# jaak-s/BayesianDataFusion.jl

Hardware: AMD Instinct MI355X
Metric: Gibbs sweeps/sec (both entities) + test RMSE, MovieLens-1M D=32 (higher is better)
Workload: dtype f64; 1 GPU; BPMF MovieLens-1M 6040x3952, 500209 training ratings (500000 held out), D=32, alpha=1.5, step = rows of both entities + hyperpriors + test prediction update (one native call); BEFORE the --warmup steps the engine's set-up runs 60 ms of full iterations whose results are discarded (device_warmup_ms); num_latent=32, burnin=5, psamples=1985, parallelism=1 GPU

## Files before the change

### bayesiandatafusion.jl_amd/csrc/bdf_gibbs.hip

```cpp
#include "bdf_common.h"
#include <algorithm>
#include <chrono>
#include <cmath>
#include <cstdio>
#include <cstdlib>
#include <map>
#include <mutex>
#include <tuple>

struct bdf_gibbs {
    bdf_ctx *rows, *hyper, *pred;
    int D;
    struct Ent {
        bdf_gibbs_entity d;
        int cur;
        hipEvent_t ev_rows = nullptr, ev_hyper = nullptr;
        hipEvent_t ev_beta = nullptr;
        bool beta_recorded = false;
        bool hyper_recorded = false;
        uint32_t epoch = 0;
        uint32_t *done_dev = nullptr;
        uint32_t done_target = 0;
        hipEvent_t t_start = nullptr, t_stop = nullptr;
        unsigned long long *span = nullptr;
    };
    std::vector<Ent> ent;
    bdf_pairs *test;
    int32_t test_entity[BDF_MAX_MODES];
    double test_mean, clamp_lo, clamp_hi, class_cut;
    double *stats_dev;
    hipEvent_t ev_pred[3] = {nullptr, nullptr, nullptr};
    uint64_t pred_at[3] = {0, 0, 0};
    uint64_t n_pred;
    uint64_t n_iter = 0;
    bdf_comm *comm;
    std::vector<bdf_gibbs_relation> rels;
    double *rel_sse = nullptr;
    uint32_t *ready_dev;
    bool polling;
    bool debug;
    double host_wait_us, host_enqueue_us;
    uint64_t n_sweeps;
};

namespace {

__global__ void k_spin(long long ticks)
{
    const long long t0 = wall_clock64();
    while (wall_clock64() - t0 < ticks) __builtin_amdgcn_s_sleep(8);
}

__global__ void k_wait_flag(const uint32_t *flag, long long max_ticks, uint32_t *timed_out)
{
    const long long t0 = wall_clock64();
    while (__hip_atomic_load(flag, __ATOMIC_RELAXED, __HIP_MEMORY_SCOPE_AGENT) == 0) {
        __builtin_amdgcn_s_sleep(8);
        if (wall_clock64() - t0 > max_ticks) { *timed_out = 1; break; }
    }
}
__global__ void k_set_flag(uint32_t *flag) { __hip_atomic_store(flag, 1u, __ATOMIC_RELEASE, __HIP_MEMORY_SCOPE_AGENT); }

int streams_concurrent(hipStream_t a, hipStream_t b, bool *yes)
{
    uint32_t *d;
    BDF_HIP(hipMalloc((void **)&d, 2 * sizeof(uint32_t)));
    struct Free { uint32_t *p; ~Free() { (void)hipFree(p); } } guard{d};
    BDF_HIP(hipMemsetAsync(d, 0, 2 * sizeof(uint32_t), a));
    BDF_HIP(hipStreamSynchronize(a)); BDF_HIP(hipStreamSynchronize(b));
    hipLaunchKernelGGL(k_wait_flag, dim3(1), dim3(1), 0, a, (const uint32_t *)d, 2000000LL, d + 1);
    hipLaunchKernelGGL(k_set_flag, dim3(1), dim3(1), 0, b, d);
    BDF_HIP(hipStreamSynchronize(a)); BDF_HIP(hipStreamSynchronize(b));
    uint32_t h[2] = {0, 0};
    BDF_HIP(hipMemcpy(h, d, sizeof(h), hipMemcpyDeviceToHost));
    *yes = h[1] == 0;
    return BDF_OK;
}

int streams_overlap(hipStream_t a, hipStream_t b, bool *yes)
{
    hipEvent_t e0, e1, e2;
    BDF_HIP(hipEventCreate(&e0)); BDF_HIP(hipEventCreate(&e1)); BDF_HIP(hipEventCreate(&e2));
    BDF_HIP(hipStreamSynchronize(a)); BDF_HIP(hipStreamSynchronize(b));
    float best = 1e9f;
    for (int rep = 0; rep < 3; rep++) {
        BDF_HIP(hipEventRecord(e0, a));
        BDF_HIP(hipStreamWaitEvent(b, e0, 0));
        hipLaunchKernelGGL(k_spin, dim3(1), dim3(64), 0, a, 6000LL);
        hipLaunchKernelGGL(k_spin, dim3(1), dim3(64), 0, b, 6000LL);
        BDF_HIP(hipEventRecord(e1, b));
        BDF_HIP(hipStreamWaitEvent(a, e1, 0));
        BDF_HIP(hipEventRecord(e2, a));
        BDF_HIP(hipEventSynchronize(e2));
        float ms = 0.f;
        BDF_HIP(hipEventElapsedTime(&ms, e0, e2));
        best = std::min(best, ms);
    }
    (void)hipEventDestroy(e0); (void)hipEventDestroy(e1); (void)hipEventDestroy(e2);
    *yes = best < 0.100f;
    return BDF_OK;
}

int pooled_stream(int device, int reserve, bool reserved, int slot, hipStream_t *out)
{
    static std::mutex mu;
    static std::map<std::tuple<int, int, int, int>, hipStream_t> pool;
    std::lock_guard<std::mutex> lock(mu);
    const auto key = std::make_tuple(device, reserve, reserved ? 1 : 0, slot);
    auto it = pool.find(key);
    if (it != pool.end()) { *out = it->second; return BDF_OK; }
    hipStream_t st;
    if (reserve <= 0) {
        BDF_HIP(hipStreamCreateWithFlags(&st, hipStreamNonBlocking));
    } else {
        hipDeviceProp_t prop;
        BDF_HIP(hipGetDeviceProperties(&prop, device));
        const int ncu = prop.multiProcessorCount, words = (ncu + 31) / 32;
        std::vector<uint32_t> mask((size_t)words, 0u);
        for (int i = 0; i < ncu; i++)
            if ((i < reserve) == reserved) mask[(size_t)(i / 32)] |= 1u << (i % 32);
        BDF_HIP(hipExtStreamCreateWithCUMask(&st, (uint32_t)words, mask.data()));
    }
    pool[key] = st;
    *out = st;
    return BDF_OK;
}

int make_side_ctx(bdf_ctx *main, const std::vector<bdf_ctx *> &apart, bool reserved, bdf_ctx **out)
{
    bdf_ctx *fallback = nullptr;
    for (int attempt = 0; attempt < 8; attempt++) {
        hipStream_t st;
        int rc = pooled_stream(main->device, main->reserve_cus, reserved, attempt + 1, &st);
        if (rc) return rc;
        if (st == main->stream) continue;
        bool taken = false;
        for (bdf_ctx *o : apart) taken = taken || o->stream == st;
        if (taken) continue;
        bdf_ctx *c;
        rc = bdf_ctx_create(main->device, (void *)st, main->seed, &c);
        if (rc) return rc;
        c->reserve_cus = main->reserve_cus;
        c->on_reserved = (reserved && main->reserve_cus > 0) ? 1 : 0;
        bool ok = true;
        if ((rc = streams_overlap(st, main->stream, &ok))) return rc;
        for (bdf_ctx *o : apart)
            if (ok && (rc = streams_overlap(st, o->stream, &ok))) return rc;
        if (ok) {
            if (fallback) bdf_ctx_destroy(fallback);
            *out = c;
            return BDF_OK;
        }
        if (!fallback) fallback = c; else bdf_ctx_destroy(c);
    }
    *out = fallback;
    return BDF_OK;
}

}

extern "C" int bdf_ctx_create_rows(int device, uint64_t seed, int reserve_cus, bdf_ctx **out)
{
    BDF_REQUIRE(out && reserve_cus >= 0 && reserve_cus % 8 == 0 && reserve_cus <= 64, BDF_ERR_ARG,
                "bdf_ctx_create_rows: reserve_cus must be 0, 8, 16, ... 64 (whole CUs per XCD)");
    int ndev = 0;
    if (hipGetDeviceCount(&ndev) != hipSuccess || ndev <= 0) {
        bdf_set_error("bdf_ctx_create_rows: no HIP device visible (this library has no CPU path)");
        return BDF_ERR_NOGPU;
    }
    BDF_REQUIRE(device >= 0 && device < ndev, BDF_ERR_ARG, "bdf_ctx_create_rows: device %d out of range", device);
    BDF_HIP(hipSetDevice(device));
    hipStream_t st;
    int rc = pooled_stream(device, reserve_cus, false, 0, &st);
    if (rc) return rc;
    bdf_ctx *c;
    if ((rc = bdf_ctx_create(device, (void *)st, seed, &c))) return rc;
    c->reserve_cus = reserve_cus;
    *out = c;
    return BDF_OK;
}

extern "C" int bdf_ctx_create_side(bdf_ctx *main_ctx, bdf_ctx *const *apart, int n_apart, int reserved, bdf_ctx **out)
{
    BDF_REQUIRE(main_ctx && out && n_apart >= 0 && (n_apart == 0 || apart), BDF_ERR_ARG, "bdf_ctx_create_side: bad argument");
    std::vector<bdf_ctx *> ap(apart, apart + n_apart);
    return make_side_ctx(main_ctx, ap, reserved != 0, out);
}

extern "C" int bdf_gibbs_create(bdf_ctx *rows_ctx, int D, int n_entities, const bdf_gibbs_entity *ents, bdf_gibbs **out)
{
    BDF_REQUIRE(rows_ctx && ents && out, BDF_ERR_ARG, "bdf_gibbs_create: NULL argument");
    BDF_REQUIRE(D >= 1 && D <= BDF_MAX_D, BDF_ERR_ARG, "bdf_gibbs_create: num_latent=%d must be in 1..%d", D, BDF_MAX_D);
    BDF_REQUIRE(n_entities >= 1 && n_entities <= 64, BDF_ERR_ARG, "bdf_gibbs_create: 1..64 entities");
    for (int j = 0; j < n_entities; j++) {
        const bdf_gibbs_entity &e = ents[j];
        BDF_REQUIRE(e.n_terms >= 1 && e.n_terms <= BDF_MAX_TERMS, BDF_ERR_ARG, "bdf_gibbs_create: entity %d takes part in %d relations (1..%d)", j, e.n_terms, BDF_MAX_TERMS);
        BDF_REQUIRE(e.sample[0] && e.sample[1] && e.sample[2] && e.mu && e.Lambda && e.mu0 && e.WI && e.sumU && e.UUt && e.prior_pack && e.draws,
                    BDF_ERR_ARG, "bdf_gibbs_create: entity %d has a NULL buffer", j);
        BDF_REQUIRE(!e.feat || (e.beta && e.uhat && e.mu_matrix && e.Tinv && e.lambda_beta), BDF_ERR_ARG,
                    "bdf_gibbs_create: entity %d has side information but a NULL beta / uhat / mu_matrix / Tinv / lambda_beta", j);
        BDF_REQUIRE(!e.feat || e.feat->m == e.N, BDF_ERR_ARG, "bdf_gibbs_create: entity %d has %lld rows but its feature matrix %lld", j,
                    (long long)e.N, e.feat ? (long long)e.feat->m : 0LL);
        for (int t = 0; t < e.n_terms; t++) {
            BDF_REQUIRE(e.terms[t].rel, BDF_ERR_ARG, "bdf_gibbs_create: entity %d term %d has no relation", j, t);
            for (int k = 0; k < e.terms[t].rel->n_modes; k++)
                BDF_REQUIRE(e.terms[t].entity_of_mode[k] >= 0 && e.terms[t].entity_of_mode[k] < n_entities, BDF_ERR_ARG,
                            "bdf_gibbs_create: entity %d term %d mode %d names entity %d", j, t, k, e.terms[t].entity_of_mode[k]);
        }
    }
    BDF_HIP(hipSetDevice(rows_ctx->device));
    bdf_gibbs *g = new bdf_gibbs();
    g->rows = rows_ctx; g->hyper = g->pred = nullptr; g->D = D; g->test = nullptr; g->stats_dev = nullptr;
    g->n_pred = 0; g->comm = nullptr; g->ready_dev = nullptr; g->polling = false;
    g->debug = false; g->host_wait_us = g->host_enqueue_us = 0.0; g->n_sweeps = 0;
    int rc;
    if ((rc = make_side_ctx(rows_ctx, {}, true, &g->hyper)) || (rc = make_side_ctx(rows_ctx, {g->hyper}, false, &g->pred))) { bdf_gibbs_destroy(g); return rc; }
    g->ready_dev = nullptr;
    g->polling = rows_ctx->reserve_cus > 0 && g->hyper->on_reserved && !getenv("BDF_NO_POLL");
    if (g->polling) {
        bool conc = false;
        if ((rc = streams_concurrent(rows_ctx->stream, g->hyper->stream, &conc))) { bdf_gibbs_destroy(g); return rc; }
        g->polling = conc;
    }
    g->debug = getenv("BDF_DEBUG") != nullptr;
    if (g->debug)
        fprintf(stderr, "[bdf_gibbs] reserve_cus=%d hyperprior stream on reserved CUs=%d polling=%d\n", rows_ctx->reserve_cus,
                g->hyper->on_reserved, (int)g->polling);
    struct Guard { bdf_gibbs *g; ~Guard() { if (g) bdf_gibbs_destroy(g); } } guard{g};
    BDF_HIP(hipMalloc((void **)&g->ready_dev, (size_t)n_entities * sizeof(uint32_t)));
    BDF_HIP(hipMemsetAsync(g->ready_dev, 0, (size_t)n_entities * sizeof(uint32_t), rows_ctx->stream));
    BDF_HIP(hipStreamSynchronize(rows_ctx->stream));
    g->ent.resize((size_t)n_entities);
    for (int j = 0; j < n_entities; j++) {
        auto &E = g->ent[(size_t)j];
        E.d = ents[j]; E.cur = 0;
        BDF_HIP(hipEventCreate(&E.ev_rows));
        BDF_HIP(hipEventCreate(&E.ev_hyper));
        if (E.d.feat) BDF_HIP(hipEventCreateWithFlags(&E.ev_beta, hipEventDisableTiming));
    }
    for (int k = 0; k < 3; k++) BDF_HIP(hipEventCreateWithFlags(&g->ev_pred[k], hipEventDisableTiming));
    if (g->polling) {
        const size_t bytes = (size_t)BDF_DONE_SHARDS * BDF_DONE_STRIDE * sizeof(uint32_t);
        for (int j = 0; j < n_entities; j++) {
            BDF_HIP(hipMalloc((void **)&g->ent[(size_t)j].done_dev, bytes));
            BDF_HIP(hipMemsetAsync(g->ent[(size_t)j].done_dev, 0, bytes, rows_ctx->stream));
        }
        BDF_HIP(hipStreamSynchronize(rows_ctx->stream));
    }
    guard.g = nullptr;
    *out = g;
    return BDF_OK;
}

extern "C" int bdf_gibbs_destroy(bdf_gibbs *g)
{
    if (!g) return BDF_OK;
    if (g->rows) (void)hipStreamSynchronize(g->rows->stream);
    if (g->debug && g->n_sweeps)
        fprintf(stderr, "[bdf_gibbs] %llu sweeps: host enqueue %.1f us per sweep, host wait for the device %.1f us per sweep\n",
                (unsigned long long)g->n_sweeps, g->host_enqueue_us / (double)g->n_sweeps, g->host_wait_us / (double)g->n_sweeps);
    for (auto &E : g->ent) {
        if (E.ev_rows) (void)hipEventDestroy(E.ev_rows);
        if (E.ev_hyper) (void)hipEventDestroy(E.ev_hyper);
        if (E.ev_beta) (void)hipEventDestroy(E.ev_beta);
        if (E.done_dev) (void)hipFree(E.done_dev);
    }
    for (int k = 0; k < 3; k++)
        if (g->ev_pred[k]) (void)hipEventDestroy(g->ev_pred[k]);
    if (g->ready_dev) (void)hipFree(g->ready_dev);
    if (g->rel_sse) (void)hipFree(g->rel_sse);
    if (g->pred) bdf_ctx_destroy(g->pred);
    if (g->hyper) bdf_ctx_destroy(g->hyper);
    delete g;
    return BDF_OK;
}

extern "C" int bdf_gibbs_contexts(bdf_gibbs *g, bdf_ctx **hyper, bdf_ctx **pred)
{
    BDF_REQUIRE(g, BDF_ERR_ARG, "bdf_gibbs_contexts: NULL argument");
    if (hyper) *hyper = g->hyper;
    if (pred) *pred = g->pred;
    return BDF_OK;
}

extern "C" int bdf_ctx_stream(const bdf_ctx *ctx, void **stream)
{
    BDF_REQUIRE(ctx && stream, BDF_ERR_ARG, "bdf_ctx_stream: NULL argument");
    *stream = (void *)ctx->stream;
    return BDF_OK;
}

extern "C" int bdf_gibbs_set_test(bdf_gibbs *g, bdf_pairs *pairs, const int32_t *entity_of_mode, double mean_value,
                                  double clamp_lo, double clamp_hi, double class_cut, double *stats_dev)
{
    BDF_REQUIRE(g && pairs && entity_of_mode && stats_dev, BDF_ERR_ARG, "bdf_gibbs_set_test: NULL argument");
    for (int k = 0; k < pairs->n_modes; k++) {
        BDF_REQUIRE(entity_of_mode[k] >= 0 && entity_of_mode[k] < (int)g->ent.size(), BDF_ERR_ARG, "bdf_gibbs_set_test: mode %d names entity %d", k, entity_of_mode[k]);
        g->test_entity[k] = entity_of_mode[k];
    }
    g->test = pairs; g->test_mean = mean_value; g->clamp_lo = clamp_lo; g->clamp_hi = clamp_hi; g->class_cut = class_cut;
    g->stats_dev = stats_dev;
    return BDF_OK;
}

extern "C" int bdf_gibbs_set_relations(bdf_gibbs *g, int n_relations, const bdf_gibbs_relation *rels)
{
    BDF_REQUIRE(g && n_relations >= 0 && (n_relations == 0 || rels), BDF_ERR_ARG, "bdf_gibbs_set_relations: bad argument");
    for (int k = 0; k < n_relations; k++) {
        const bdf_gibbs_relation &r = rels[k];
        BDF_REQUIRE(r.rel && (r.alpha_dev || r.probit), BDF_ERR_ARG, "bdf_gibbs_set_relations: relation %d has no handle or no alpha_dev", k);
        BDF_REQUIRE(!(r.alpha_sample || r.feat) || r.train, BDF_ERR_ARG, "bdf_gibbs_set_relations: relation %d needs its observations as pairs (train)", k);
        BDF_REQUIRE(!r.feat || (r.beta && r.linear), BDF_ERR_ARG, "bdf_gibbs_set_relations: relation %d has features but no beta / linear buffer", k);
        BDF_REQUIRE(!r.feat_test || r.test_baseline, BDF_ERR_ARG, "bdf_gibbs_set_relations: relation %d has test features but no baseline buffer", k);
        BDF_REQUIRE(!r.probit || (!r.feat && !r.alpha_sample), BDF_ERR_ARG, "bdf_gibbs_set_relations: relation %d: the probit model takes neither relation features nor a sampled alpha", k);
        BDF_REQUIRE(!r.probit || (r.train && r.linear), BDF_ERR_ARG, "bdf_gibbs_set_relations: relation %d: the probit model needs its observations as pairs (train) and a linear buffer", k);
        BDF_REQUIRE(!r.censor || (!r.probit && !r.feat), BDF_ERR_ARG, "bdf_gibbs_set_relations: relation %d: the censored model takes neither the probit model nor relation features", k);
        BDF_REQUIRE(!r.censor || (r.train && r.linear), BDF_ERR_ARG, "bdf_gibbs_set_relations: relation %d: the censored model needs its observations as pairs (train) and a linear buffer", k);
        BDF_REQUIRE(!r.interval || (!r.probit && !r.censor && !r.feat), BDF_ERR_ARG, "bdf_gibbs_set_relations: relation %d: the interval model takes neither the probit model, censoring flags nor relation features", k);
        BDF_REQUIRE(!r.interval || (r.train && r.linear), BDF_ERR_ARG, "bdf_gibbs_set_relations: relation %d: the interval model needs its observations as pairs (train) and a linear buffer", k);
        BDF_REQUIRE(!r.ordinal || (r.interval && r.ordinal_codes && !g->comm), BDF_ERR_ARG, "bdf_gibbs_set_relations: relation %d: the ordinal model needs the interval model's bounds and the observations' levels, on one rank", k);
        BDF_REQUIRE(r.robust_nu == 0.0 || (r.robust_nu >= 1.0 && std::isfinite(r.robust_nu)), BDF_ERR_ARG,
                    "bdf_gibbs_set_relations: relation %d: robust_nu=%g must be 0 (off) or at least 1 and finite", k, r.robust_nu);
        BDF_REQUIRE(!(r.robust_nu > 0.0) || (r.train && r.obs_precision), BDF_ERR_ARG, "bdf_gibbs_set_relations: relation %d: the robust model needs its observations as pairs (train) and an obs_precision buffer", k);
        BDF_REQUIRE(!r.obs_precision || (!r.probit && !r.censor && !r.interval && !r.ordinal && !r.feat), BDF_ERR_ARG,
                    "bdf_gibbs_set_relations: relation %d: observation weights take neither the probit, censored, interval or ordinal model nor relation features", k);
        BDF_REQUIRE(!r.obs_precision || !g->comm, BDF_ERR_ARG, "bdf_gibbs_set_relations: relation %d: observation weights need one rank", k);
        BDF_REQUIRE(r.pg_model >= 0 && r.pg_model <= 2, BDF_ERR_ARG, "bdf_gibbs_set_relations: relation %d: pg_model=%d must be 0 (none), 1 (logit) or 2 (counts)", k, r.pg_model);
        BDF_REQUIRE(!r.pg_model || (r.train && r.linear && r.obs_precision), BDF_ERR_ARG,
                    "bdf_gibbs_set_relations: relation %d: a Polya-Gamma model needs its observations as pairs (train), a linear and an obs_precision buffer", k);
        BDF_REQUIRE(!r.pg_model || (!r.probit && !r.censor && !r.interval && !r.ordinal && r.robust_nu == 0.0 && !r.feat && !r.alpha_sample && !g->comm), BDF_ERR_ARG,
                    "bdf_gibbs_set_relations: relation %d: a Polya-Gamma model takes neither the probit, censored, interval, ordinal or robust model, relation features, a sampled alpha nor a communicator", k);
        BDF_REQUIRE(r.pg_model != 2 || (r.pg_r >= 1.0 && r.pg_r <= 2147483648.0 && r.pg_r == std::floor(r.pg_r)), BDF_ERR_ARG,
                    "bdf_gibbs_set_relations: relation %d: pg_r=%g must be an integer, at least 1", k, r.pg_r);
        for (int m = 0; m < r.rel->n_modes; m++)
            BDF_REQUIRE(r.entity_of_mode[m] >= 0 && r.entity_of_mode[m] < (int)g->ent.size(), BDF_ERR_ARG,
                        "bdf_gibbs_set_relations: relation %d mode %d names entity %d", k, m, r.entity_of_mode[m]);
    }
    g->rels.assign(rels, rels + n_relations);
    if (n_relations > 0 && !g->rel_sse) BDF_HIP(hipMalloc((void **)&g->rel_sse, 8 * sizeof(double)));
    return BDF_OK;
}

namespace {
const bdf_gibbs_relation *relation_of(const bdf_gibbs *g, const bdf_rel *rel)
{
    for (const auto &r : g->rels)
        if (r.rel == rel) return &r;
    return nullptr;
}

inline bool draws_latent(const bdf_gibbs_relation &r) { return r.probit || r.censor || r.interval || r.pg_model; }

int update_relations(bdf_gibbs *g)
{
    bdf_ctx *R = g->rows;
    const int D = g->D;
    int rc;
    for (const auto &r : g->rels) {
        if (!r.alpha_sample && !r.feat && !draws_latent(r) && !(r.robust_nu > 0.0)) continue;
        const double *fac[BDF_MAX_MODES];
        for (int m = 0; m < r.rel->n_modes; m++) {
            const auto &O = g->ent[(size_t)r.entity_of_mode[m]];
            fac[m] = O.d.sample[O.cur];
        }
        if (r.robust_nu > 0.0 && (rc = bdf_robust_draw(R, r.train, D, fac, r.mean_value, 0.0, r.alpha_dev, r.robust_nu, r.rel_tag, r.obs_precision,
                                                      r.alpha_sample ? g->rel_sse + 1 : nullptr)))
            return rc;
        if (r.alpha_sample) {
            if (r.obs_precision) rc = r.robust_nu > 0.0 ? BDF_OK : bdf_pairs_weighted_sse(R, r.train, D, fac, r.mean_value, r.obs_precision, g->rel_sse + 1);
            else rc = bdf_predict_sse(R, r.train, D, fac, r.mean_value, nullptr, g->rel_sse);
            if (rc) return rc;
            if (g->comm && (rc = bdf_sum_ranks(R, g->comm, g->rel_sse + 1, 1))) return rc;
            if ((rc = bdf_sample_alpha(R, r.alpha_lambda0, r.alpha_nu0, r.nnz, g->rel_sse + 1, r.rel_tag, r.alpha_dev))) return rc;
        }
        if (r.probit && (rc = bdf_probit_draw(R, r.train, D, fac, r.mean_value, r.rel_tag, r.linear + r.first_obs, nullptr))) return rc;
        if (r.pg_model && (rc = bdf_pg_draw(R, r.train, D, fac, r.mean_value, r.pg_model, r.pg_r, r.rel_tag, r.obs_precision, r.linear + r.first_obs)))
            return rc;
        if (r.censor && (rc = bdf_censored_draw(R, r.train, r.censor, D, fac, r.mean_value, 0.0, r.alpha_dev, r.rel_tag, r.linear + r.first_obs, nullptr)))
            return rc;
        if (r.ordinal && (rc = bdf_ordinal_step(R, r.ordinal, r.train, r.ordinal_codes, D, fac, r.mean_value, 0.0, r.alpha_dev, r.rel_tag, -1,
                                                const_cast<double *>(r.interval))))
            return rc;
        if (r.interval && (rc = bdf_interval_draw(R, r.train, r.interval, D, fac, r.mean_value, 0.0, r.alpha_dev, r.rel_tag, r.linear + r.first_obs, nullptr)))
            return rc;
        if (r.feat) {
            if ((rc = bdf_sample_beta_rel_impl(R, g->comm, r.feat, r.train, r.first_obs, D, fac, r.mean_value, 1.0, r.alpha_dev, r.lambda_beta,
                                               r.rel_tag, r.beta, r.linear + r.first_obs, nullptr)))
                return rc;
            if (g->comm) {
                if ((rc = bdf_allgather_block(R, g->comm, r.linear, sizeof(double) * (size_t)r.obs_block)) || (rc = bdf_allgather_join(R, g->comm))) return rc;
            }
            if (r.feat_test) {
                for (int k = 0; k < 3; k++)
                    if (g->n_pred > (uint64_t)k) BDF_HIP(hipStreamWaitEvent(R->stream, g->ev_pred[(g->n_pred - 1 - (uint64_t)k) % 3], 0));
                if ((rc = bdf_feat_linear(R, r.feat_test, r.beta, r.mean_value, r.test_baseline))) return rc;
            }
        }
    }
    return BDF_OK;
}
}

extern "C" int bdf_gibbs_set_comm(bdf_gibbs *g, bdf_comm *comm)
{
    BDF_REQUIRE(g, BDF_ERR_ARG, "bdf_gibbs_set_comm: NULL argument");
    g->comm = comm;
    return BDF_OK;
}

namespace {
double hyper_nu(const bdf_gibbs_entity &e) { return e.nu0 + ((e.feat && e.full_lambda_u) ? (double)e.feat->n : 0.0); }
}

extern "C" int bdf_gibbs_rows_only(bdf_gibbs *g, int entity, uint32_t sweep)
{
    BDF_REQUIRE(g && entity >= 0 && entity < (int)g->ent.size(), BDF_ERR_ARG, "bdf_gibbs_rows_only: bad argument");
    bdf_ctx *R = g->rows;
    auto &E = g->ent[(size_t)entity];
    const bdf_gibbs_entity &e = E.d;
    R->sweep_host = sweep;
    bdf_term terms[BDF_MAX_TERMS];
    for (int t = 0; t < e.n_terms; t++) {
        terms[t].rel = e.terms[t].rel; terms[t].mode = e.terms[t].mode; terms[t]._pad = 0;
        terms[t].alpha = e.terms[t].alpha; terms[t].mean_value = e.terms[t].mean_value; terms[t].linear_values = nullptr;
        terms[t].alpha_dev = nullptr; terms[t].obs_precision = nullptr;
        if (const bdf_gibbs_relation *gr = relation_of(g, e.terms[t].rel)) {
            terms[t].alpha_dev = gr->probit ? nullptr : gr->alpha_dev;
            terms[t].linear_values = (gr->feat || draws_latent(*gr)) ? gr->linear : nullptr;
            if (gr->probit) terms[t].alpha = 1.0;
            terms[t].obs_precision = gr->obs_precision;
        }
        for (int k = 0; k < BDF_MAX_MODES; k++) terms[t].factors[k] = nullptr;
        for (int k = 0; k < e.terms[t].rel->n_modes; k++) {
            const auto &O = g->ent[(size_t)e.terms[t].entity_of_mode[k]];
            terms[t].factors[k] = O.d.sample[O.cur];
        }
    }
    const int nxt = (E.cur + 1) % 3;
    const int nch = e.terms[0].rel->chunks;
    int rc;
    for (int c = 0; c < nch; c++)
        if ((rc = bdf_sample_rows(R, g->D, e.N, e.n_terms, terms, e.feat ? e.mu_matrix : e.mu, e.feat ? 1 : 0, e.Lambda, e.tag, c, nch,
                                  e.sample[nxt], (E.hyper_recorded && !e.feat) ? e.prior_pack : nullptr)))
            return rc;
    E.cur = nxt;
    return BDF_OK;
}

extern "C" int bdf_gibbs_warm_device(bdf_gibbs *g, double milliseconds)
{
    BDF_REQUIRE(g && milliseconds >= 0.0 && milliseconds <= 10000.0, BDF_ERR_ARG, "bdf_gibbs_warm_device: bad argument");
    if (milliseconds <= 0.0) return BDF_OK;
    bdf_ctx *R = g->rows;
    const int D = g->D, n = (int)g->ent.size();
    int rc;
    if ((rc = bdf_gibbs_sync(g))) return rc;
    struct Piece { void *p; size_t bytes; bool sample; int ent; };
    std::vector<Piece> pieces;
    std::vector<char> flags;
    const size_t DD = (size_t)D * D * sizeof(double), Dv = (size_t)D * sizeof(double);
    for (int j = 0; j < n; j++) {
        auto &E = g->ent[(size_t)j];
        const bdf_gibbs_entity &e = E.d;
        pieces.push_back({e.sample[E.cur], (size_t)e.N * Dv, true, j});
        pieces.push_back({e.mu, Dv, false, j}); pieces.push_back({e.Lambda, DD, false, j});
        pieces.push_back({e.sumU, Dv, false, j}); pieces.push_back({e.UUt, DD, false, j});
        if (e.params) pieces.push_back({e.params, Dv + DD, false, j});
        pieces.push_back({e.prior_pack, (size_t)bdf_prior_pack_doubles(D) * sizeof(double), false, j});
        pieces.push_back({e.draws, DD + Dv, false, j});
        if (e.feat) {
            pieces.push_back({e.beta, (size_t)e.feat->n * Dv, false, j});
            pieces.push_back({e.uhat, (size_t)e.N * Dv, false, j});
            pieces.push_back({e.mu_matrix, (size_t)e.N * Dv, false, j});
            pieces.push_back({e.Tinv, DD, false, j});
            pieces.push_back({e.lambda_beta, sizeof(double), false, j});
            if (e.cg_iters) pieces.push_back({e.cg_iters, (size_t)D * sizeof(int32_t), false, j});
        }
        flags.push_back(E.hyper_recorded ? 1 : 0); flags.push_back(E.beta_recorded ? 1 : 0);
    }
    if (g->stats_dev) pieces.push_back({g->stats_dev, 4 * sizeof(double), false, 0});
    for (const auto &r : g->rels) {
        if (r.alpha_dev) pieces.push_back({r.alpha_dev, sizeof(double), false, 0});
        if (r.feat) {
            int world = 1, rk = 0;
            if (g->comm) (void)bdf_comm_size(g->comm, &rk, &world);
            pieces.push_back({r.beta, (size_t)r.feat->n * sizeof(double), false, 0});
            pieces.push_back({r.linear, (size_t)r.obs_block * (size_t)world * sizeof(double), false, 0});
            if (r.feat_test) pieces.push_back({r.test_baseline, (size_t)r.feat_test->m * sizeof(double), false, 0});
        }
        if (draws_latent(r)) pieces.push_back({r.linear + r.first_obs, (size_t)r.train->n * sizeof(double), false, 0});
        if (r.robust_nu > 0.0 || r.pg_model) pieces.push_back({r.obs_precision, (size_t)r.train->n * sizeof(double), false, 0});
        if (r.ordinal) {
            pieces.push_back({r.ordinal->state_dev, r.ordinal->state_doubles * sizeof(double), false, 0});
            pieces.push_back({const_cast<double *>(r.interval), (size_t)r.train->n * 2 * sizeof(double), false, 0});
        }
    }
    size_t total = 0;
    for (auto &pc : pieces) total += (pc.bytes + 255) & ~(size_t)255;
    char *snap = nullptr;
    BDF_HIP(hipMalloc((void **)&snap, std::max<size_t>(total, 256)));
    struct Free { char *p; ~Free() { if (p) (void)hipFree(p); } } guard{snap};
    size_t off = 0;
    for (auto &pc : pieces) {
        BDF_HIP(hipMemcpyAsync(snap + off, pc.p, pc.bytes, hipMemcpyDeviceToDevice, R->stream));
        off += (pc.bytes + 255) & ~(size_t)255;
    }
    BDF_HIP(hipStreamSynchronize(R->stream));
    const uint32_t keep = R->sweep_host;
    int64_t fixed = 0;
    const auto t0 = std::chrono::steady_clock::now();
    int64_t k = 0;
    rc = BDF_OK;
    while (!rc) {
        for (int b = 0; b < 8 && !rc; b++, k++) rc = bdf_gibbs_sweep(g, 0xfffe0000u + (uint32_t)(k & 0xffff), g->test ? 3 : -1);
        if (rc) break;
        if (g->comm && fixed == 0) {
            if ((rc = bdf_gibbs_sync(g))) break;
            const double per_iter = std::chrono::duration<double, std::milli>(std::chrono::steady_clock::now() - t0).count() / 8.0;
            const double mine = std::max(8.0, std::min(20000.0, milliseconds / std::max(per_iter, 1e-3)));
            int rank = 0, world = 1;
            if ((rc = bdf_comm_size(g->comm, &rank, &world))) break;
            void *sv;
            if ((rc = bdf_scratch(R, ((size_t)world + 1) * sizeof(double), &sv))) break;
            double *cnt = (double *)sv;
            BDF_HIP(hipMemcpyAsync(cnt, &mine, sizeof(double), hipMemcpyHostToDevice, R->stream));
            if ((rc = bdf_sum_ranks_into(R, g->comm, cnt, 1, cnt + 1))) break;
            double sum = 0.0;
            BDF_HIP(hipMemcpyAsync(&sum, cnt, sizeof(double), hipMemcpyDeviceToHost, R->stream));
            BDF_HIP(hipStreamSynchronize(R->stream));
            fixed = std::max<int64_t>(8, (int64_t)(sum / (double)world + 0.5));
        }
        if (fixed ? k >= fixed : std::chrono::duration<double, std::milli>(std::chrono::steady_clock::now() - t0).count() >= milliseconds) break;
    }
    const int rc_sync = bdf_gibbs_sync(g);
    if (!rc) rc = rc_sync;
    off = 0;
    for (auto &pc : pieces) {
        void *dst = pc.sample ? (void *)g->ent[(size_t)pc.ent].d.sample[g->ent[(size_t)pc.ent].cur] : pc.p;
        BDF_HIP(hipMemcpyAsync(dst, snap + off, pc.bytes, hipMemcpyDeviceToDevice, R->stream));
        off += (pc.bytes + 255) & ~(size_t)255;
    }
    for (int j = 0; j < n; j++) {
        g->ent[(size_t)j].hyper_recorded = flags[(size_t)2 * j] != 0;
        g->ent[(size_t)j].beta_recorded = flags[(size_t)2 * j + 1] != 0;
    }
    BDF_HIP(hipStreamSynchronize(R->stream));
    R->sweep_host = g->hyper->sweep_host = g->pred->sweep_host = keep;
    return rc;
}

extern "C" int bdf_gibbs_recorded(const bdf_gibbs *g, int entity, int *hyper, int *beta)
{
    BDF_REQUIRE(g && entity >= 0 && entity < (int)g->ent.size() && hyper && beta, BDF_ERR_ARG, "bdf_gibbs_recorded: bad argument");
    *hyper = g->ent[(size_t)entity].hyper_recorded ? 1 : 0;
    *beta = g->ent[(size_t)entity].beta_recorded ? 1 : 0;
    return BDF_OK;
}

extern "C" int bdf_gibbs_set_recorded(bdf_gibbs *g, int entity, int hyper, int beta)
{
    BDF_REQUIRE(g && entity >= 0 && entity < (int)g->ent.size(), BDF_ERR_ARG, "bdf_gibbs_set_recorded: bad argument");
    g->ent[(size_t)entity].hyper_recorded = hyper != 0;
    g->ent[(size_t)entity].beta_recorded = beta != 0;
    return BDF_OK;
}

extern "C" int bdf_gibbs_time_rows(bdf_gibbs *g, int entity, void *start, void *stop)
{
    BDF_REQUIRE(g && entity >= 0 && entity < (int)g->ent.size(), BDF_ERR_ARG, "bdf_gibbs_time_rows: bad entity");
    g->ent[(size_t)entity].t_start = (hipEvent_t)start;
    g->ent[(size_t)entity].t_stop = (hipEvent_t)stop;
    return BDF_OK;
}

extern "C" int bdf_gibbs_span_rows(bdf_gibbs *g, int entity, void *slot_dev)
{
    BDF_REQUIRE(g && entity >= 0 && entity < (int)g->ent.size(), BDF_ERR_ARG, "bdf_gibbs_span_rows: bad entity");
    g->ent[(size_t)entity].span = (unsigned long long *)slot_dev;
    return BDF_OK;
}

extern "C" int bdf_gibbs_current(const bdf_gibbs *g, int entity, int *buffer)
{
    BDF_REQUIRE(g && buffer && entity >= 0 && entity < (int)g->ent.size(), BDF_ERR_ARG, "bdf_gibbs_current: bad argument");
    *buffer = g->ent[(size_t)entity].cur;
    return BDF_OK;
}

extern "C" int bdf_gibbs_sweep(bdf_gibbs *g, uint32_t sweep, int predict_phase)
{
    BDF_REQUIRE(g, BDF_ERR_ARG, "bdf_gibbs_sweep: NULL argument");
    bdf_ctx *R = g->rows, *H = g->hyper, *P = g->pred;
    const int D = g->D, n = (int)g->ent.size();
    int rc;
    R->sweep_host = H->sweep_host = P->sweep_host = sweep;
    constexpr uint64_t pred_lag = 3;
    const auto t_in = std::chrono::steady_clock::now();
    for (uint64_t back = 1; back <= std::min<uint64_t>(g->n_pred, 3); back++) {
        const uint64_t k = (g->n_pred - back) % 3;
        if (g->pred_at[k] + pred_lag <= g->n_iter) {
            hipError_t st = hipErrorNotReady;
            const auto t_spin = std::chrono::steady_clock::now();
            while ((st = hipEventQuery(g->ev_pred[k])) == hipErrorNotReady &&
                   std::chrono::duration<double, std::micro>(std::chrono::steady_clock::now() - t_spin).count() < 400.0) { }
            if (st == hipErrorNotReady) st = hipEventSynchronize(g->ev_pred[k]);
            BDF_HIP(st);
            break;
        }
    }
    const auto t_go = std::chrono::steady_clock::now();
    bool draws_in_chain = !g->comm;
    for (int j = 0; j < n; j++) draws_in_chain = draws_in_chain && g->ent[(size_t)j].d.N <= 16384;
    if (!draws_in_chain && n <= BDF_DRAWS_BATCH) {
        int64_t Ns[BDF_DRAWS_BATCH]; double nus[BDF_DRAWS_BATCH]; uint32_t tags[BDF_DRAWS_BATCH]; double *outs[BDF_DRAWS_BATCH];
        for (int j = 0; j < n; j++) {
            const bdf_gibbs_entity &e = g->ent[(size_t)j].d;
            Ns[j] = e.n_real; nus[j] = hyper_nu(e); tags[j] = e.tag; outs[j] = e.draws;
        }
        if ((rc = bdf_hyper_draws_batch(H, D, n, Ns, nus, tags, outs))) return rc;
    }
    if (!g->rels.empty() && (rc = update_relations(g))) return rc;
    for (int j = 0; j < n; j++) {
        auto &E = g->ent[(size_t)j];
        const bdf_gibbs_entity &e = E.d;
        static const bool poll_with_comm = getenv("BDF_POLL_WITH_COMM") != nullptr;
        const bool poll = g->polling && (!g->comm || poll_with_comm) && E.hyper_recorded && !e.feat;
        if (E.hyper_recorded && !poll) BDF_HIP(hipStreamWaitEvent(R->stream, E.ev_hyper, 0));
        if (e.feat && (rc = bdf_uhat(R, e.feat, D, e.beta, e.mu, e.uhat, e.mu_matrix))) return rc;
        if (!draws_in_chain && n > BDF_DRAWS_BATCH && (rc = bdf_hyper_draws(H, D, e.n_real, hyper_nu(e), e.tag, e.draws))) return rc;
        bdf_term terms[BDF_MAX_TERMS];
        for (int t = 0; t < e.n_terms; t++) {
            terms[t].rel = e.terms[t].rel; terms[t].mode = e.terms[t].mode; terms[t]._pad = 0;
            terms[t].alpha = e.terms[t].alpha; terms[t].mean_value = e.terms[t].mean_value; terms[t].linear_values = nullptr;
            terms[t].alpha_dev = nullptr; terms[t].obs_precision = nullptr;
            if (const bdf_gibbs_relation *gr = relation_of(g, e.terms[t].rel)) {
                terms[t].alpha_dev = gr->probit ? nullptr : gr->alpha_dev;
                terms[t].linear_values = (gr->feat || draws_latent(*gr)) ? gr->linear : nullptr;
                if (gr->probit) terms[t].alpha = 1.0;
                terms[t].obs_precision = gr->obs_precision;
            }
            for (int k = 0; k < BDF_MAX_MODES; k++) terms[t].factors[k] = nullptr;
            for (int k = 0; k < e.terms[t].rel->n_modes; k++) {
                const auto &O = g->ent[(size_t)e.terms[t].entity_of_mode[k]];
                terms[t].factors[k] = O.d.sample[O.cur];
            }
        }
        const int nxt = (E.cur + 1) % 3;
        hipEvent_t done = E.t_stop ? E.t_stop : E.ev_rows;
        const int nch = e.terms[0].rel->chunks;
        const bool counter = E.done_dev && draws_in_chain && g->polling && !g->comm && !e.feat && nch == 1 && !E.t_stop;
        const bool pred_waits = j == n - 1 && g->test && predict_phase >= 0;
        bool by_counter = false;
        for (int c = 0; c < nch; c++) {
            R->time_start = (c == 0) ? E.t_start : nullptr;
            R->rows_span = E.span;
            R->time_stop = (c == nch - 1 && !g->comm && !(counter && !pred_waits)) ? done : nullptr;
            if (poll) { R->rows_ready = g->ready_dev + j; R->rows_ready_want = E.epoch; }
            if (counter) R->rows_done = E.done_dev;
            if ((rc = bdf_sample_rows(R, D, e.N, e.n_terms, terms, e.feat ? e.mu_matrix : e.mu, e.feat ? 1 : 0, e.Lambda, e.tag, c, nch,
                                      e.sample[nxt], (E.hyper_recorded && !e.feat) ? e.prior_pack : nullptr)))
                return rc;
            if (counter && R->rows_done_added >= 0) { by_counter = true; E.done_target += (uint32_t)R->rows_done_added; }
            if (g->comm && (rc = bdf_allgather_rows(R, g->comm, D, e.N, e.sample[nxt], c, nch))) return rc;
        }
        if (g->comm) {
            if ((rc = bdf_allgather_join(R, g->comm))) return rc;
            BDF_HIP(hipEventRecord(done, R->stream));
        } else if (counter && !pred_waits && !by_counter) {
            BDF_HIP(hipEventRecord(done, R->stream));
        }
        E.t_start = E.t_stop = nullptr;
        E.span = nullptr;
        E.cur = nxt;
        if (by_counter) { H->hyper_wait = E.done_dev; H->hyper_wait_target = E.done_target; }
        else BDF_HIP(hipStreamWaitEvent(H->stream, done, 0));
        H->hyper_fuse = true;
        const double *Tinv = e.WI;
        if (e.feat && e.full_lambda_u) {
            if (E.beta_recorded) BDF_HIP(hipStreamWaitEvent(H->stream, E.ev_beta, 0));
            if ((rc = bdf_hyper_feature_terms(H, D, e.feat->n, e.beta, e.WI, e.lambda_beta, e.Tinv))) return rc;
            Tinv = e.Tinv;
        }
        if ((rc = g->comm ? bdf_hyper_sums_ranks(H, g->comm, D, e.N, nch, e.sample[E.cur], e.feat ? e.uhat : nullptr, e.sumU, e.UUt)
                          : bdf_hyper_sums(H, D, e.N, e.sample[E.cur], e.feat ? e.uhat : nullptr, e.sumU, e.UUt)))
            return rc;
        H->hyper_chain_draws = draws_in_chain ? e.draws : nullptr;
        H->time_h_stop = E.ev_hyper;
        H->hyper_ready = g->ready_dev + j;
        H->hyper_ready_value = ++E.epoch;
        if ((rc = bdf_hyper_sample(H, D, e.n_real, e.sumU, e.UUt, e.mu0, e.b0, Tinv, hyper_nu(e), e.tag, e.mu, e.Lambda, e.params, e.prior_pack, e.draws)))
            return rc;
        E.hyper_recorded = true;
        if (j == n - 1 && g->test && predict_phase >= 0) BDF_HIP(hipStreamWaitEvent(P->stream, done, 0));
    }
    for (int j = 0; j < n; j++) {
        auto &E = g->ent[(size_t)j];
        const bdf_gibbs_entity &e = E.d;
        if (!e.feat) continue;
        BDF_HIP(hipStreamWaitEvent(R->stream, E.ev_hyper, 0));
        if ((rc = bdf_sample_beta_ranks(R, g->comm, e.feat, D, e.sample[E.cur], e.mu, e.Lambda, e.lambda_beta, e.use_ff, e.tol, 0,
                                        e.sample_lambda_beta, e.lb_nu, e.lb_mu, e.tag, e.beta, nullptr, e.cg_iters)))
            return rc;
        BDF_HIP(hipEventRecord(E.ev_beta, R->stream));
        E.beta_recorded = true;
    }
    if (g->test && predict_phase >= 0) {
        const double *fac[BDF_MAX_MODES];
        for (int k = 0; k < g->test->n_modes; k++) {
            const auto &O = g->ent[(size_t)g->test_entity[k]];
            fac[k] = O.d.sample[O.cur];
        }
        if ((rc = predict_phase == 3 ? bdf_predict_sse(P, g->test, D, fac, g->test_mean, nullptr, g->stats_dev)
                                     : bdf_predict_update(P, g->test, D, fac, g->test_mean, predict_phase, g->clamp_lo, g->clamp_hi, g->class_cut, g->stats_dev)))
            return rc;
        BDF_HIP(hipEventRecord(g->ev_pred[g->n_pred % 3], P->stream));
        g->pred_at[g->n_pred % 3] = g->n_iter;
        g->n_pred++;
    }
    g->n_iter++;
    if (g->debug) {
        g->host_wait_us += std::chrono::duration<double, std::micro>(t_go - t_in).count();
        g->host_enqueue_us += std::chrono::duration<double, std::micro>(std::chrono::steady_clock::now() - t_go).count();
        g->n_sweeps++;
    }
    return BDF_OK;
}

extern "C" int bdf_gibbs_sync(bdf_gibbs *g)
{
    BDF_REQUIRE(g, BDF_ERR_ARG, "bdf_gibbs_sync: NULL argument");
    int rc;
    if ((rc = bdf_ctx_sync(g->pred)) || (rc = bdf_ctx_sync(g->hyper))) return rc;
    return bdf_ctx_sync(g->rows);
}
```

### bayesiandatafusion.jl_amd/csrc/k_update_runs.hip

```cpp
#include "bdf_common.h"
#include "predict.h"

namespace {

constexpr int RUN = 16;
constexpr int NB = 4;

__global__ __launch_bounds__(256) void k_update_runs(PredArgs a)
{
    const int tid = threadIdx.x, sub = tid & 7;
    const int ks = a.sorted_mode, ko = 1 - ks;
    const int32_t *ids_s = a.ids + (int64_t)ks * a.n, *ids_o = a.ids + (int64_t)ko * a.n;
    const double *fs = a.fac[ks], *fo = a.fac[ko];
    const bool live = sub * 4 < a.D;
    const int eoff = live ? sub * 4 : 0;
    const int64_t p0 = ((int64_t)blockIdx.x * 32 + tid / 8) * RUN;
    int32_t cur = -1;
    double4 srow = {0.0, 0.0, 0.0, 0.0};
    double keep[2] = {0.0, 0.0};
#pragma unroll
    for (int q = 0; q < 2; q++) {
        if (p0 + 8 * q >= a.n) break;
        const int64_t pm = p0 + 8 * q + sub < a.n ? p0 + 8 * q + sub : a.n - 1;
        const int32_t my_s = ids_s[pm], my_o = ids_o[pm];
#pragma unroll
        for (int u0 = 0; u0 < 8; u0 += NB) {
            double4 orow[NB];
#pragma unroll
            for (int u = 0; u < NB; u++) orow[u] = *(const double4 *)(fo + (int64_t)__shfl(my_o, u0 + u, 8) * a.D + eoff);
#pragma unroll
            for (int u = 0; u < NB; u++) {
                const int32_t is = __shfl(my_s, u0 + u, 8);
                if (is != cur) { srow = *(const double4 *)(fs + (int64_t)is * a.D + eoff); cur = is; }
                double s = live ? (srow.x * orow[u].x + srow.y * orow[u].y) + (srow.z * orow[u].z + srow.w * orow[u].w) : 0.0;
                s += __shfl_xor(s, 4); s += __shfl_xor(s, 2); s += __shfl_xor(s, 1);
                if (sub == u0 + u) keep[q] = s;
            }
        }
    }
    __builtin_amdgcn_sched_barrier(0);
    double st[4] = {0.0, 0.0, 0.0, 0.0};
#pragma unroll
    for (int q = 0; q < 2; q++) {
        PairState ps;
        const int64_t p = p0 + 8 * q + sub;
        ps.ok = p < a.n;
        ps.pm = ps.ok ? p : a.n - 1;
        ps.po = ps.pm;
        ps.base = a.mean;
        ps.y = a.values[ps.pm];
        ps.av = 0.0; ps.sv = 0.0;
        if (a.phase == 2) { ps.av = a.avg[ps.pm]; ps.sv = a.sq[ps.pm]; }
        pair_finish(a, ps, keep[q], st);
    }
    block_stats(a, st);
}

}

int bdf_update_runs(bdf_ctx *ctx, const bdf_pairs *p, int D, const double *const *factors, double mean_value, int phase, double count,
                    double clamp_lo, double clamp_hi, double class_cut, double *stats_out)
{
    PredArgs a;
    int rc = fill("bdf_predict_update", ctx, p, D, factors, a);
    if (rc) return rc;
    BDF_REQUIRE(a.sorted_mode >= 0 && a.n_modes == 2 && (D & 3) == 0 && D <= 32 && a.linear == nullptr && phase >= 0 && phase <= 2,
                BDF_ERR_ARG, "bdf_update_runs: not the sorted two-mode update");
    if (a.n == 0) return BDF_OK;
    a.mean = mean_value; a.avg = p->avg_dev; a.sq = p->sq_dev; a.phase = phase; a.count = count;
    a.clamp_lo = clamp_lo; a.clamp_hi = clamp_hi; a.cut = class_cut; a.stats = stats_out;
    a.orig = nullptr; a.out = nullptr;
    const int nblocks = (int)((a.n + 32 * RUN - 1) / (32 * RUN));
    return launch_reduced(ctx, nblocks, a.partial, a.stats,
                          [&] { hipLaunchKernelGGL(k_update_runs, dim3(nblocks), dim3(256), 0, ctx->stream, a); });
}
```

Baseline: 13150 sweeps/s.

## Gate prediction on row-done counter via side-stream kernel; shrink update blocks to single waves

When rows finish via a device counter, a small gate kernel on a new reserved side stream now spins on the done counters and then records the rows event. The prediction stream waits on that event instead of the rows stream's completion event, so the rows stream no longer records a stop event just for prediction. Separately, the test-prediction update kernel is split into 64-thread single-wave blocks with a VGPR cap, reducing each block with shuffles only, and a one-block final kernel sums the partials. This trades an extra spinning kernel and one extra launch for avoiding block-level syncs and a host-side reduction helper.

```diff
diff --git a/bayesiandatafusion.jl_amd/csrc/bdf_gibbs.hip b/bayesiandatafusion.jl_amd/csrc/bdf_gibbs.hip
--- a/bayesiandatafusion.jl_amd/csrc/bdf_gibbs.hip
+++ b/bayesiandatafusion.jl_amd/csrc/bdf_gibbs.hip
@@ -10,6 +10,7 @@
 
 struct bdf_gibbs {
     bdf_ctx *rows, *hyper, *pred;
+    bdf_ctx *gate = nullptr;
     int D;
     struct Ent {
         bdf_gibbs_entity d;
@@ -61,6 +62,19 @@
 }
 __global__ void k_set_flag(uint32_t *flag) { __hip_atomic_store(flag, 1u, __ATOMIC_RELEASE, __HIP_MEMORY_SCOPE_AGENT); }
 
+__global__ __launch_bounds__(64) void k_rows_gate(const uint32_t *done, uint32_t target, int *flag)
+{
+    int spins = 0;
+    for (;;) {
+        uint32_t v = __hip_atomic_load(done + BDF_DONE_STRIDE * threadIdx.x, __ATOMIC_RELAXED, __HIP_MEMORY_SCOPE_AGENT);
+#pragma unroll
+        for (int off = 32; off >= 1; off >>= 1) v += __shfl_xor(v, off);
+        if ((int32_t)(v - target) >= 0) break;
+        __builtin_amdgcn_s_sleep(8);
+        if (++spins > (1 << 22)) { if (threadIdx.x == 0) atomicOr_system(flag, 16); break; }
+    }
+}
+
 int streams_concurrent(hipStream_t a, hipStream_t b, bool *yes)
 {
     uint32_t *d;
@@ -222,6 +236,8 @@
         if ((rc = streams_concurrent(rows_ctx->stream, g->hyper->stream, &conc))) { bdf_gibbs_destroy(g); return rc; }
         g->polling = conc;
     }
+    if (g->polling && (rc = make_side_ctx(rows_ctx, {g->hyper, g->pred}, true, &g->gate))) { bdf_gibbs_destroy(g); return rc; }
+    if (g->polling && !g->gate) g->polling = false;
     g->debug = getenv("BDF_DEBUG") != nullptr;
     if (g->debug)
         fprintf(stderr, "[bdf_gibbs] reserve_cus=%d hyperprior stream on reserved CUs=%d polling=%d\n", rows_ctx->reserve_cus,
@@ -269,6 +285,7 @@
         if (g->ev_pred[k]) (void)hipEventDestroy(g->ev_pred[k]);
     if (g->ready_dev) (void)hipFree(g->ready_dev);
     if (g->rel_sse) (void)hipFree(g->rel_sse);
+    if (g->gate) { (void)hipStreamSynchronize(g->gate->stream); bdf_ctx_destroy(g->gate); }
     if (g->pred) bdf_ctx_destroy(g->pred);
     if (g->hyper) bdf_ctx_destroy(g->hyper);
     delete g;
@@ -654,7 +671,7 @@
         for (int c = 0; c < nch; c++) {
             R->time_start = (c == 0) ? E.t_start : nullptr;
             R->rows_span = E.span;
-            R->time_stop = (c == nch - 1 && !g->comm && !(counter && !pred_waits)) ? done : nullptr;
+            R->time_stop = (c == nch - 1 && !g->comm && !counter) ? done : nullptr;
             if (poll) { R->rows_ready = g->ready_dev + j; R->rows_ready_want = E.epoch; }
             if (counter) R->rows_done = E.done_dev;
             if ((rc = bdf_sample_rows(R, D, e.N, e.n_terms, terms, e.feat ? e.mu_matrix : e.mu, e.feat ? 1 : 0, e.Lambda, e.tag, c, nch,
@@ -666,7 +683,7 @@
         if (g->comm) {
             if ((rc = bdf_allgather_join(R, g->comm))) return rc;
             BDF_HIP(hipEventRecord(done, R->stream));
-        } else if (counter && !pred_waits && !by_counter) {
+        } else if (counter && !by_counter) {
             BDF_HIP(hipEventRecord(done, R->stream));
         }
         E.t_start = E.t_stop = nullptr;
@@ -691,7 +708,12 @@
         if ((rc = bdf_hyper_sample(H, D, e.n_real, e.sumU, e.UUt, e.mu0, e.b0, Tinv, hyper_nu(e), e.tag, e.mu, e.Lambda, e.params, e.prior_pack, e.draws)))
             return rc;
         E.hyper_recorded = true;
-        if (j == n - 1 && g->test && predict_phase >= 0) BDF_HIP(hipStreamWaitEvent(P->stream, done, 0));
+        if (pred_waits && by_counter) {
+            hipExtLaunchKernelGGL(k_rows_gate, dim3(1), dim3(64), 0, g->gate->stream, nullptr, E.ev_rows, 0, (const uint32_t *)E.done_dev,
+                                  E.done_target, H->flag_dev);
+            BDF_HIP(hipGetLastError());
+            BDF_HIP(hipStreamWaitEvent(P->stream, E.ev_rows, 0));
+        } else if (pred_waits) BDF_HIP(hipStreamWaitEvent(P->stream, done, 0));
     }
     for (int j = 0; j < n; j++) {
         auto &E = g->ent[(size_t)j];
diff --git a/bayesiandatafusion.jl_amd/csrc/k_update_runs.hip b/bayesiandatafusion.jl_amd/csrc/k_update_runs.hip
--- a/bayesiandatafusion.jl_amd/csrc/k_update_runs.hip
+++ b/bayesiandatafusion.jl_amd/csrc/k_update_runs.hip
@@ -5,8 +5,9 @@
 
 constexpr int RUN = 16;
 constexpr int NB = 4;
+#define UPD_VGPR_HALF 48
 
-__global__ __launch_bounds__(256) void k_update_runs(PredArgs a)
+__global__ __launch_bounds__(64) __attribute__((amdgpu_num_vgpr(UPD_VGPR_HALF))) void k_update_runs(PredArgs a)
 {
     const int tid = threadIdx.x, sub = tid & 7;
     const int ks = a.sorted_mode, ko = 1 - ks;
@@ -14,7 +15,7 @@
     const double *fs = a.fac[ks], *fo = a.fac[ko];
     const bool live = sub * 4 < a.D;
     const int eoff = live ? sub * 4 : 0;
-    const int64_t p0 = ((int64_t)blockIdx.x * 32 + tid / 8) * RUN;
+    const int64_t p0 = ((int64_t)blockIdx.x * 8 + tid / 8) * RUN;
     int32_t cur = -1;
     double4 srow = {0.0, 0.0, 0.0, 0.0};
     double keep[2] = {0.0, 0.0};
@@ -53,7 +54,35 @@
         if (a.phase == 2) { ps.av = a.avg[ps.pm]; ps.sv = a.sq[ps.pm]; }
         pair_finish(a, ps, keep[q], st);
     }
-    block_stats(a, st);
+#pragma unroll
+    for (int q = 0; q < 4; q++)
+#pragma unroll
+        for (int off = 32; off >= 1; off >>= 1) st[q] += __shfl_xor(st[q], off);
+    if (tid == 0) {
+        double *w = a.partial + (int64_t)blockIdx.x * 4;
+        w[0] = st[0]; w[1] = st[1]; w[2] = st[2]; w[3] = st[3];
+    }
+}
+
+__global__ __launch_bounds__(256) void k_update_waves_final(int nblocks, const double *wave, double *stats)
+{
+    __shared__ double red[4][4];
+    const int tid = threadIdx.x;
+    double v[4] = {0.0, 0.0, 0.0, 0.0};
+    for (int b = tid; b < nblocks; b += 256) {
+        const double *w = wave + (int64_t)b * 16;
+#pragma unroll
+        for (int q = 0; q < 4; q++) v[q] += w[q] + w[4 + q] + w[8 + q] + w[12 + q];
+    }
+#pragma unroll
+    for (int q = 0; q < 4; q++) {
+        double x = v[q];
+#pragma unroll
+        for (int off = 32; off >= 1; off >>= 1) x += __shfl_xor(x, off);
+        if ((tid & 63) == 0) red[q][tid >> 6] = x;
+    }
+    __syncthreads();
+    if (tid < 4) stats[tid] = red[tid][0] + red[tid][1] + red[tid][2] + red[tid][3];
 }
 
 }
@@ -71,6 +100,12 @@
     a.clamp_lo = clamp_lo; a.clamp_hi = clamp_hi; a.cut = class_cut; a.stats = stats_out;
     a.orig = nullptr; a.out = nullptr;
     const int nblocks = (int)((a.n + 32 * RUN - 1) / (32 * RUN));
-    return launch_reduced(ctx, nblocks, a.partial, a.stats,
-                          [&] { hipLaunchKernelGGL(k_update_runs, dim3(nblocks), dim3(256), 0, ctx->stream, a); });
+    void *sc;
+    rc = bdf_scratch(ctx, (size_t)nblocks * 16 * sizeof(double), &sc);
+    if (rc) return rc;
+    a.partial = (double *)sc;
+    hipLaunchKernelGGL(k_update_runs, dim3(4 * (unsigned)nblocks), dim3(64), 0, ctx->stream, a);
+    hipLaunchKernelGGL(k_update_waves_final, dim3(1), dim3(256), 0, ctx->stream, nblocks, (const double *)a.partial, a.stats);
+    BDF_HIP(hipGetLastError());
+    return BDF_OK;
 }
```

Result: faster. 13450 sweeps/s, median of 6 (+2.3%).
